# westlake-repl/IDvs.MoRec

Hardware: AMD Instinct MI355X
Metric: user-sequences/sec end-to-end train step, SASRec+BERT-base (higher is better)
Workload: dtype fp16

## Files before the change

idvs/morec_amd/_lib.py:

```python
from __future__ import annotations

import ctypes as C
import os

import torch

_HERE = os.path.dirname(os.path.abspath(__file__))
LIB_PATH = os.environ.get("MOREC_HIP_LIB") or os.path.join(_HERE, "libmorec_hip.so")

F32, BF16, F16 = 0, 1, 2
ACT_NONE, ACT_GELU, ACT_RELU = 0, 1, 2
DACT_MUL = 3


class MorecError(RuntimeError):
    pass


class GemmDesc(C.Structure):
    _fields_ = [("M", C.c_int), ("N", C.c_int), ("K", C.c_int), ("lda", C.c_int), ("ldb", C.c_int), ("ldc", C.c_int),
                ("in_dtype", C.c_int), ("out_dtype", C.c_int), ("act", C.c_int), ("dact", C.c_int),
                ("accumulate", C.c_int), ("split_k", C.c_int), ("alpha", C.c_float), ("aux_deriv", C.c_int)]


class GemmPlanInfo(C.Structure):
    _fields_ = [("family", C.c_int), ("mode", C.c_int), ("tile_rows", C.c_int), ("tile_cols", C.c_int), ("ngroup", C.c_int),
                ("colsum_fused", C.c_int), ("family_name", C.c_char_p)]


class AttnDesc(C.Structure):
    _fields_ = [("n_seq", C.c_int), ("T", C.c_int), ("n_heads", C.c_int), ("dh", C.c_int), ("causal", C.c_int),
                ("scale", C.c_float), ("mask_value", C.c_float), ("dtype", C.c_int), ("p_drop", C.c_float),
                ("seed", C.c_uint64), ("cu_seqlens", C.c_void_p), ("total_rows", C.c_int), ("spare_rows_max", C.c_int)]


class TransposeItem(C.Structure):
    _fields_ = [("src", C.c_void_p), ("dst", C.c_void_p), ("rows", C.c_int), ("cols", C.c_int), ("ld_src", C.c_int),
                ("ld_dst", C.c_int), ("tile0", C.c_int), ("reserved", C.c_int)]


class CeDesc(C.Structure):
    _fields_ = [("B", C.c_int), ("S", C.c_int), ("D", C.c_int), ("Nc", C.c_int), ("col_offset", C.c_int),
                ("dtype", C.c_int), ("dE_fp32", C.c_int), ("ws_from_fwd", C.c_int)]


class StepParams(C.Structure):
    _fields_ = [("step", C.c_int32), ("found_inf", C.c_int32), ("growth_tracker", C.c_int32), ("skipped", C.c_int32),
                ("loss_scale", C.c_float), ("inv_scale", C.c_float), ("bc1", C.c_float), ("bc2", C.c_float), ("apply", C.c_int32),
                ("pad0", C.c_int32), ("drop_seed", C.c_uint64), ("drop_seed_mixed", C.c_uint64), ("reserved", C.c_int32 * 2)]


class SwinAttnDesc(C.Structure):
    _fields_ = [("n_img", C.c_int), ("H", C.c_int), ("W", C.c_int), ("window", C.c_int), ("shift", C.c_int),
                ("heads", C.c_int), ("dh", C.c_int), ("scale", C.c_float), ("dtype", C.c_int)]


_P = C.c_void_p
_SIGS = {
    "morec_strerror": (C.c_char_p, [C.c_int]),
    "morec_version": (C.c_int, []),
    "morec_tuning_set": (C.c_int, [C.c_char_p, C.c_int]),
    "morec_det_scratch_reserve": (C.c_int, [C.c_size_t, C.c_void_p]),
    "morec_stream_wait_stream": (C.c_int, [_P, _P]),
    "morec_fold_defer_begin": (C.c_int, [_P]),
    "morec_fold_defer_active": (C.c_int, []),
    "morec_fold_flush": (C.c_int, [_P]),
    "morec_fold_defer_end": (C.c_int, []),
    "morec_fold_stats": (C.c_int, [_P]),
    "morec_gemm_nt": (C.c_int, [C.POINTER(GemmDesc), _P, _P, _P, _P, _P, _P, _P]),
    "morec_gemm_nt_colsum": (C.c_int, [C.POINTER(GemmDesc), _P, _P, _P, _P, _P, _P, _P, _P, _P]),
    "morec_gemm_colsum_workspace_bytes": (C.c_size_t, [C.c_int, C.c_int]),
    "morec_gemm_plan": (C.c_int, [C.POINTER(GemmDesc), C.c_int, C.c_int, C.c_int, C.c_int, C.c_int, C.POINTER(GemmPlanInfo)]),
    "morec_gemm_tn": (C.c_int, [_P, _P, _P, C.c_int, C.c_int, C.c_int, C.c_int, C.c_int, C.c_int, C.c_int, C.c_int, C.c_int, _P, _P]),
    "morec_gemm_tn_workspace_bytes": (C.c_size_t, [C.c_int, C.c_int, C.c_int]),
    "morec_mlp_dact_recompute_supported": (C.c_int, [C.c_int, C.c_int, C.c_int, C.c_int]),
    "morec_mlp_dact_recompute_workspace_bytes": (C.c_size_t, [C.c_int]),
    "morec_mlp_dact_recompute": (C.c_int, [_P, _P, _P, _P, _P, _P, _P, _P, C.c_int, C.c_int, C.c_int, C.c_int, _P]),
    "morec_transpose": (C.c_int, [_P, _P, C.c_int, C.c_int, C.c_int, C.c_int, C.c_int, C.c_int, _P]),
    "morec_transpose_batch": (C.c_int, [_P, C.c_int, C.c_int, C.c_int, _P]),
    "morec_cast": (C.c_int, [_P, _P, C.c_size_t, C.c_int, C.c_int, _P]),
    "morec_split_bf16x3": (C.c_int, [_P, _P, C.c_int, C.c_int, C.c_int, C.c_int, C.c_int, _P]),
    "morec_act_bwd": (C.c_int, [_P, _P, _P, C.c_size_t, C.c_int, C.c_int, _P]),
    "morec_scaled_sum": (C.c_int, [_P, _P, _P, _P, C.c_size_t, C.c_float, C.c_int, _P]),
    "morec_colsum": (C.c_int, [_P, _P, C.c_int, C.c_int, C.c_int, C.c_int, _P]),
    "morec_layernorm_fwd": (C.c_int, [_P, _P, _P, _P, C.c_int, _P, _P, C.c_float, _P, _P, _P, _P, C.c_int, C.c_int,
                                      C.c_int, C.c_float, C.c_uint64, C.c_float, C.c_uint64, _P, C.c_int, _P]),
    "morec_layernorm_bwd": (C.c_int, [_P, _P, _P, _P, _P, _P, _P, _P, _P, _P, _P, C.c_int, C.c_int, C.c_int, C.c_float,
                                      C.c_uint64, C.c_float, C.c_uint64, _P, _P, C.c_int, _P]),
    "morec_layernorm_fwd_res32": (C.c_int, [_P, _P, _P, _P, C.c_int, _P, _P, C.c_float, _P, _P, _P, _P, _P, C.c_int, C.c_int,
                                            C.c_int, C.c_float, C.c_uint64, C.c_float, C.c_uint64, _P]),
    "morec_layernorm_fwd_res32_pre": (C.c_int, [_P, _P, _P, _P, _P, _P, _P, _P, _P, C.c_float, _P, _P, _P, _P, C.c_int, C.c_int, C.c_int,
                                                C.c_float, C.c_uint64, _P]),
    "morec_layernorm_bwd_res32": (C.c_int, [_P, _P, _P, _P, _P, _P, _P, _P, _P, _P, _P, C.c_int, C.c_int, C.c_int, C.c_float,
                                            C.c_uint64, C.c_float, C.c_uint64, _P]),
    "morec_pos_grad": (C.c_int, [_P, _P, C.c_int, C.c_int, C.c_int, C.c_int, _P]),
    "morec_attn_fwd": (C.c_int, [C.POINTER(AttnDesc), _P, _P, _P, _P]),
    "morec_attn_bwd": (C.c_int, [C.POINTER(AttnDesc), _P, _P, _P, _P, _P]),
    "morec_attn_bwd_dbias": (C.c_int, [C.POINTER(AttnDesc), _P, _P, _P, _P, C.c_int, _P, _P, C.c_size_t, _P]),
    "morec_bert_embed_fwd": (C.c_int, [_P, _P, _P, _P, _P, _P, C.c_float, _P, _P, _P, _P, C.c_int, C.c_int, C.c_int,
                                       C.c_int, C.c_float, C.c_uint64, _P]),
    "morec_bert_embed_bwd": (C.c_int, [_P, _P, _P, _P, _P, C.c_int, C.c_int, C.c_int, C.c_int, C.c_int, _P, _P]),
    "morec_gather_rows": (C.c_int, [_P, _P, _P, C.c_int, C.c_int, C.c_int, _P]),
    "morec_scatter_add_rows": (C.c_int, [_P, _P, _P, C.c_int, C.c_int, C.c_int, C.c_int, _P]),
    "morec_indexed_rows_copy": (C.c_int, [_P, _P, _P, _P, C.c_int, C.c_int, C.c_int, _P]),
    "morec_strided_rows_copy": (C.c_int, [_P, _P, C.c_int, C.c_int, C.c_int, C.c_int, C.c_int, _P]),
    "morec_inbatch_ce_workspace_bytes": (C.c_size_t, [C.POINTER(CeDesc)]),
    "morec_inbatch_ce_fwd": (C.c_int, [C.POINTER(CeDesc), _P, _P, _P, _P, _P, _P, _P, _P, _P, _P, _P, _P]),
    "morec_inbatch_ce_bwd": (C.c_int, [C.POINTER(CeDesc), _P, _P, _P, _P, _P, _P, _P, _P, _P, C.c_float, _P, _P, _P,
                                       _P]),
    "morec_bce_fwd": (C.c_int, [_P, _P, _P, _P, _P, C.c_int, C.c_int, C.c_int, C.c_int, _P]),
    "morec_bce_bwd": (C.c_int, [_P, _P, _P, _P, _P, _P, _P, C.c_int, C.c_int, C.c_int, C.c_int, _P]),
    "morec_adamw": (C.c_int, [_P, _P, _P, _P, _P, C.c_size_t, C.c_float, C.c_float, C.c_float, C.c_float, C.c_float,
                              C.c_int, C.c_float, _P]),
    "morec_dropout_seed_source": (C.c_int, [_P]),
    "morec_step_params_init": (C.c_int, [_P, C.c_float, C.c_int, _P]),
    "morec_grad_check_finite": (C.c_int, [_P, C.c_size_t, _P, _P]),
    "morec_step_decide": (C.c_int, [_P, C.c_float, C.c_float, C.c_float, C.c_float, C.c_int, C.c_int, _P]),
    "morec_adamw_sp": (C.c_int, [_P, _P, _P, _P, _P, C.c_int, C.c_size_t, C.c_float, C.c_float, C.c_float, C.c_float, C.c_float, _P, _P]),
    "morec_eval_rank": (C.c_int, [_P, _P, _P, C.c_int, _P, _P, _P, C.c_int, C.c_int, C.c_int, _P]),
    "morec_eval_rank_cand": (C.c_int, [_P, _P, _P, C.c_int, _P, C.c_int, _P, _P, _P, C.c_int, C.c_int, C.c_int, _P]),
    "morec_eval_topk": (C.c_int, [_P, _P, _P, C.c_int, C.c_int, C.c_int, _P, _P, _P, C.c_size_t, C.c_int, C.c_int, C.c_int, _P]),
    "morec_eval_topk_ws_bytes": (C.c_size_t, [C.c_int, C.c_int, C.c_int, C.c_int]),
    "morec_eval_topk_max_k": (C.c_int, []),
    "morec_dropout_keep_mask": (C.c_int, [_P, C.c_size_t, C.c_float, C.c_uint64, _P]),
    "morec_probe": (C.c_int, [_P, _P]),
    "morec_swin_attn_fwd": (C.c_int, [C.POINTER(SwinAttnDesc), _P, _P, _P, _P]),
    "morec_swin_attn_bwd": (C.c_int, [C.POINTER(SwinAttnDesc), _P, _P, _P, _P, _P, _P, _P]),
    "morec_swin_attn_bwd_dbias": (C.c_int, [C.POINTER(SwinAttnDesc), _P, _P, _P, _P, _P, _P, _P, _P, C.c_size_t, _P]),
    "morec_swin_bias_expand": (C.c_int, [_P, _P, C.c_int, C.c_int, _P]),
    "morec_swin_bias_reduce": (C.c_int, [_P, _P, C.c_int, C.c_int, _P]),
    "morec_swin_patchify": (C.c_int, [_P, _P, C.c_int, C.c_int, C.c_int, C.c_int, C.c_int, C.c_int, _P]),
    "morec_swin_patchify_u8": (C.c_int, [_P, _P, C.c_int, C.c_int, C.c_int, C.c_int, C.c_int, C.c_float, C.c_float, C.c_int, _P]),
    "morec_swin_merge": (C.c_int, [_P, _P, C.c_int, C.c_int, C.c_int, C.c_int, C.c_int, C.c_int, _P]),
    "morec_swin_pool_fwd": (C.c_int, [_P, _P, C.c_int, C.c_int, C.c_int, C.c_int, _P]),
    "morec_swin_pool_bwd": (C.c_int, [_P, _P, C.c_int, C.c_int, C.c_int, C.c_int, _P]),
    "morec_bias_residual": (C.c_int, [_P, _P, _P, _P, C.c_int, _P, C.c_int, C.c_int, C.c_int, _P]),
    "morec_droppath_scale": (C.c_int, [_P, C.c_int, C.c_float, C.c_uint64, _P]),
    "morec_image_resize_u8": (C.c_int, [_P, _P, _P, _P, C.c_int, C.c_int, _P]),
    "morec_comm_available": (C.c_int, []),
    "morec_comm_unique_id": (C.c_int, [_P]),
    "morec_comm_create": (C.c_int, [C.POINTER(_P), _P, C.c_int, C.c_int]),
    "morec_comm_destroy": (C.c_int, [_P]),
    "morec_comm_last_error": (C.c_char_p, [_P]),
    "morec_comm_all_gather": (C.c_int, [_P, _P, _P, C.c_size_t, _P]),
    "morec_comm_reduce_scatter_f32": (C.c_int, [_P, _P, _P, C.c_size_t, _P]),
    "morec_comm_all_reduce_f32": (C.c_int, [_P, _P, C.c_size_t, _P]),
}

EXPORTS = tuple(_SIGS)
_lib = None


def lib():
    global _lib
    if _lib is None:
        if not os.path.exists(LIB_PATH):
            raise MorecError(f"{LIB_PATH} not found: build it with `python -c 'import __graft_entry__ as g; g.build()'` "
                             "or `make -C idvs/morec_amd/csrc` -- there is no CPU/PyTorch fallback path")
        h = C.CDLL(LIB_PATH)
        for name, (res, args) in _SIGS.items():
            fn = getattr(h, name)
            fn.restype, fn.argtypes = res, args
        _lib = h
        h.morec_tuning_set(b"deterministic", int(env_flag("MOREC_DETERMINISTIC")))
    return _lib


def env_flag(name: str) -> bool:
    return os.environ.get(name, "0").strip().lower() not in ("", "0", "false", "no", "off")


def check(rc: int, what: str):
    if rc != 0:
        msg = lib().morec_strerror(rc)
        raise MorecError(f"{what} failed: rc={rc} ({msg.decode() if msg else '?'})")
```

idvs/morec_amd/csrc/gemm_tn8p.hip:

```cpp
#include "gemm_core.hpp"
#include "gemm_args.hpp"


namespace {
typedef __attribute__((ext_vector_type(16))) float f32x16_t;
typedef __attribute__((ext_vector_type(4))) unsigned int u32x4_t;
typedef __attribute__((ext_vector_type(4))) short s16x4_t;
typedef __attribute__((ext_vector_type(8))) short s16x8_t;
typedef __attribute__((address_space(3))) s16x4_t* lds_s16x4_ptr;

constexpr int TT = 64;
constexpr int ROWB = 256;
constexpr int HALF_BYTES = TT * ROWB;
constexpr int OP_BYTES = 2 * HALF_BYTES;
constexpr int BUF_BYTES = 2 * OP_BYTES;
constexpr int LDS_MAIN = 2 * BUF_BYTES;
constexpr int SLICE = 4096;
constexpr int LDS_TOTAL = LDS_MAIN + 8 * SLICE;
constexpr int THREADS = 512;

struct TnArgs8 {
    const bf16* DY;
    const bf16* X;
    float* out;
    int M, N, K, ldy, ldx, ldo, mchunk, tiles_n, tiles_k, zs;
    size_t slab_stride;
};

template <int N>
__device__ __forceinline__ void vm_wait() {
    asm volatile("s_waitcnt vmcnt(%0)" ::"n"(N) : "memory");
}
__device__ __forceinline__ void pin() { __builtin_amdgcn_sched_barrier(0); }
__device__ __forceinline__ void bar() {
    pin();
    __builtin_amdgcn_s_barrier();
    pin();
}
template <int REM, int W1, int W0>
__device__ __forceinline__ void vm_wait_tail() {
    vm_wait<(REM >= 2 ? 8 : (REM == 1 ? W1 : W0))>();
}

struct Ctx {
    __amdgpu_buffer_rsrc_t ry, rx;
    uint32_t y1[2], y2[2], x1[2], x2[2];
    int tok[2];
    int dpiece;
    int ay[2], ax;
    uint32_t vmask;
};

__device__ __forceinline__ void dma2(__amdgpu_buffer_rsrc_t rs, const uint32_t (&o)[2], const int (&tok)[2], int left, int soff, char* dst) {
    const uint32_t o0 = tok[0] < left ? o[0] : 0x80000000u;
    const uint32_t o1 = tok[1] < left ? o[1] : 0x80000000u;
    __builtin_amdgcn_raw_ptr_buffer_load_lds(rs, (lptr_t)dst, 16, o0, soff, 0, 0);
    __builtin_amdgcn_raw_ptr_buffer_load_lds(rs, (lptr_t)(dst + 1024), 16, o1, soff, 0, 0);
}

__device__ __forceinline__ bf16x8_t tr_frag(const char* smem, int addr, int ks) {
    const s16x4_t lo = __builtin_amdgcn_ds_read_tr16_b64_v4i16((lds_s16x4_ptr)(smem + addr + (16 * ks) * ROWB));
    const s16x4_t hi = __builtin_amdgcn_ds_read_tr16_b64_v4i16((lds_s16x4_ptr)(smem + addr + (16 * ks + 4) * ROWB));
    const s16x8_t v = {lo[0], lo[1], lo[2], lo[3], hi[0], hi[1], hi[2], hi[3]};
    return __builtin_bit_cast(bf16x8_t, v);
}

template <typename T16, int N0, int KQ, bool SKIP>
__device__ __forceinline__ void mfma_quadrant(f32x16_t (&acc)[4][2], const bf16x8_t (&fy)[2][4], const bf16x8_t (&fx)[4], uint32_t vm) {
    if constexpr (SKIP) {
        if (!(vm & (16u << KQ))) return;
        const bool a = (vm >> N0) & 1u, b = (vm >> (N0 + 1)) & 1u;
        if (!(a && b)) {
            if (!(a || b)) return;
            __builtin_amdgcn_s_setprio(1);
            if (a) {
#pragma unroll
                for (int ks = 0; ks < 4; ++ks) acc[N0][KQ] = h16<T16>::mma32(fx[ks], fy[0][ks], acc[N0][KQ]);
            } else {
#pragma unroll
                for (int ks = 0; ks < 4; ++ks) acc[N0 + 1][KQ] = h16<T16>::mma32(fx[ks], fy[1][ks], acc[N0 + 1][KQ]);
            }
            __builtin_amdgcn_s_setprio(0);
            return;
        }
    }
    __builtin_amdgcn_s_setprio(1);
#pragma unroll
    for (int ks = 0; ks < 4; ++ks)
#pragma unroll
        for (int ni = 0; ni < 2; ++ni)
            acc[N0 + ni][KQ] = h16<T16>::mma32(fx[ks], fy[ni][ks], acc[N0 + ni][KQ]);
    __builtin_amdgcn_s_setprio(0);
}

template <typename T16, int REM, bool SKIP>
__device__ __forceinline__ void stage(char* smem, const Ctx& c, int cb, int soy, int sox, int dy_step, int dx_step, int left,
                                      f32x16_t (&acc)[4][2]) {
    char* cur = smem + cb;
    char* oth = smem + (cb ^ BUF_BYTES);
    bf16x8_t fy[2][4], fx0[4], fx1[4];
    const int ay0 = cb + c.ay[0], ay1 = cb + c.ay[1], ax = cb + OP_BYTES + c.ax;
#pragma unroll
    for (int ks = 0; ks < 4; ++ks) fx0[ks] = tr_frag(smem, ax, ks);
#pragma unroll
    for (int ks = 0; ks < 4; ++ks) {
        fy[0][ks] = tr_frag(smem, ay0, ks);
        fy[1][ks] = tr_frag(smem, ay1, ks);
    }
    if constexpr (REM >= 1) dma2(c.rx, c.x2, c.tok, left - TT, sox + dx_step, oth + OP_BYTES + HALF_BYTES + c.dpiece);
    pin();
    vm_wait_tail<REM, 8, 2>();
    bar();
    mfma_quadrant<T16, 0, 0, SKIP>(acc, fy, fx0, c.vmask);
    bar();
#pragma unroll
    for (int ks = 0; ks < 4; ++ks) fx1[ks] = tr_frag(smem, ax + HALF_BYTES, ks);
    if constexpr (REM >= 1) dma2(c.ry, c.y2, c.tok, left - TT, soy + dy_step, oth + HALF_BYTES + c.dpiece);
    pin();
    vm_wait_tail<REM, 8, 0>();
    bar();
    mfma_quadrant<T16, 0, 1, SKIP>(acc, fy, fx1, c.vmask);
    bar();
#pragma unroll
    for (int ks = 0; ks < 4; ++ks) {
        fy[0][ks] = tr_frag(smem, ay0 + HALF_BYTES, ks);
        fy[1][ks] = tr_frag(smem, ay1 + HALF_BYTES, ks);
    }
    if constexpr (REM >= 2) dma2(c.ry, c.y1, c.tok, left - 2 * TT, soy + 2 * dy_step, cur + c.dpiece);
    pin();
    vm_wait_tail<REM, 6, 0>();
    bar();
    mfma_quadrant<T16, 2, 1, SKIP>(acc, fy, fx1, c.vmask);
    bar();
    if constexpr (REM >= 2) dma2(c.rx, c.x1, c.tok, left - 2 * TT, sox + 2 * dx_step, cur + OP_BYTES + c.dpiece);
    pin();
    vm_wait_tail<REM, 4, 0>();
    bar();
    mfma_quadrant<T16, 2, 0, SKIP>(acc, fy, fx0, c.vmask);
    bar();
}

template <typename T16, bool SKIP>
__device__ __forceinline__ void tn_body(const TnArgs8& p, char* smem, const bf16* __restrict__ DYt, const bf16* __restrict__ Xt, int n0, int k0,
                                        int mbeg, int mend, float* __restrict__ dst) {
    const int lane = threadIdx.x & 63;
    const int wave = __builtin_amdgcn_readfirstlane(threadIdx.x >> 6);
    const int wr = wave >> 2, wc = wave & 3;
    const int nt = (mend - mbeg + TT - 1) / TT;
    Ctx c;
    {
#pragma unroll
        for (int j = 0; j < 2; ++j) {
            const int t = 8 * wave + 4 * j + (lane >> 4);
            const int lc = (lane & 15) ^ (4 * (t & 3));
            const int ycol = (lc < 8 ? lc * 8 : 128 + (lc - 8) * 8);
            const int xcol = (lc >> 2) * 64 + (lc & 3) * 8;
            c.tok[j] = t;
            c.y1[j] = (uint32_t)(t * p.ldy + min(n0 + ycol, p.N - 8) - n0) * 2u;
            c.y2[j] = (uint32_t)(t * p.ldy + min(n0 + ycol + 64, p.N - 8) - n0) * 2u;
            c.x1[j] = (uint32_t)(t * p.ldx + min(k0 + xcol, p.K - 8) - k0) * 2u;
            c.x2[j] = (uint32_t)(t * p.ldx + min(k0 + xcol + 32, p.K - 8) - k0) * 2u;
        }
        const long ybytes = (long)(p.M - mbeg) * p.ldy * 2, xbytes = (long)(p.M - mbeg) * p.ldx * 2;
        c.ry = __builtin_amdgcn_make_buffer_rsrc((void*)DYt, 0, (int)min(ybytes, 0x7fffffffL), 0x00020000);
        c.rx = __builtin_amdgcn_make_buffer_rsrc((void*)Xt, 0, (int)min(xbytes, 0x7fffffffL), 0x00020000);
        c.dpiece = 8 * wave * ROWB;
        const int rr = (lane & 15) >> 2, cgrp = (lane >> 4) & 1, h = lane >> 5;
        const int rowoff = (8 * h + rr) * ROWB + 8 * (lane & 3);
#pragma unroll
        for (int cg = 0; cg < 2; ++cg) c.ay[cg] = rowoff + (((wr * 4 + cg * 2 + cgrp) ^ (2 * rr)) << 5);
        c.ax = rowoff + (((wc * 2 + cgrp) ^ (2 * rr)) << 5);
        uint32_t vm = 0;
#pragma unroll
        for (int i = 0; i < 4; ++i) vm |= (n0 + wr * 128 + i * 32 < p.N) ? (1u << i) : 0u;
#pragma unroll
        for (int j = 0; j < 2; ++j) vm |= (k0 + wc * 64 + j * 32 < p.K) ? (16u << j) : 0u;
        c.vmask = __builtin_amdgcn_readfirstlane(vm);
    }
    const int dy_step = TT * p.ldy * 2, dx_step = TT * p.ldx * 2;
    const int left0 = mend - mbeg;
    dma2(c.ry, c.y1, c.tok, left0, 0, smem + c.dpiece);
    dma2(c.rx, c.x1, c.tok, left0, 0, smem + OP_BYTES + c.dpiece);
    dma2(c.rx, c.x2, c.tok, left0, 0, smem + OP_BYTES + HALF_BYTES + c.dpiece);
    dma2(c.ry, c.y2, c.tok, left0, 0, smem + HALF_BYTES + c.dpiece);
    dma2(c.ry, c.y1, c.tok, left0 - TT, dy_step, smem + BUF_BYTES + c.dpiece);
    dma2(c.rx, c.x1, c.tok, left0 - TT, dx_step, smem + BUF_BYTES + OP_BYTES + c.dpiece);
    pin();

    f32x16_t acc[4][2];
#pragma unroll
    for (int i = 0; i < 4; ++i)
#pragma unroll
        for (int j = 0; j < 2; ++j)
#pragma unroll
            for (int v = 0; v < 16; ++v) acc[i][j][v] = 0.f;
    vm_wait<8>();
    bar();
    if (wr == 1) bar();
    int cb = 0, t = 0;
    for (; t < nt - 2; ++t) {
        stage<T16, 2, SKIP>(smem, c, cb, t * dy_step, t * dx_step, dy_step, dx_step, left0 - t * TT, acc);
        cb ^= BUF_BYTES;
    }
    stage<T16, 1, SKIP>(smem, c, cb, t * dy_step, t * dx_step, dy_step, dx_step, left0 - t * TT, acc);
    stage<T16, 0, SKIP>(smem, c, cb ^ BUF_BYTES, (t + 1) * dy_step, (t + 1) * dx_step, dy_step, dx_step, left0 - (t + 1) * TT, acc);
    if (wr == 0) bar();

    const int r5 = lane & 31, hh = lane >> 5;
    char* ws = smem + LDS_MAIN + wave * SLICE;
    const int rs_row = lane >> 3, rs_slot = lane & 7;
    const int rs_off = rs_row * 128 + ((rs_slot ^ (rs_row & 7)) << 4);
    const int nrows = min(256, p.N - n0);
    const long obytes = (long)nrows * p.ldo * 4;
    const __amdgpu_buffer_rsrc_t ro = __builtin_amdgcn_make_buffer_rsrc((void*)(dst + (size_t)n0 * p.ldo), 0, (int)min(obytes, 0x7fffffffL), 0x00020000);
    auto wfence = [&]() {
        __builtin_amdgcn_fence(__ATOMIC_RELEASE, "wavefront");
        __builtin_amdgcn_wave_barrier();
        __builtin_amdgcn_fence(__ATOMIC_ACQUIRE, "wavefront");
    };
#pragma unroll
    for (int Ni = 0; Ni < 4; ++Ni) {
#pragma unroll
        for (int Ki = 0; Ki < 2; ++Ki) {
            pin();
#pragma unroll
            for (int g = 0; g < 4; ++g) {
                const int slot = 2 * g + hh;
                *reinterpret_cast<float4*>(ws + r5 * 128 + ((slot ^ (r5 & 7)) << 4)) =
                    make_float4(acc[Ni][Ki][4 * g], acc[Ni][Ki][4 * g + 1], acc[Ni][Ki][4 * g + 2], acc[Ni][Ki][4 * g + 3]);
            }
            wfence();
            u32x4_t q[4];
#pragma unroll
            for (int i = 0; i < 4; ++i) q[i] = *reinterpret_cast<const u32x4_t*>(ws + rs_off + i * 1024);
            const int kcol = k0 + wc * 64 + Ki * 32 + rs_slot * 4;
            const uint32_t lo = kcol < p.K ? (uint32_t)((rs_row * p.ldo + kcol) * 4) : 0x80000000u;
#pragma unroll
            for (int i = 0; i < 4; ++i)
                __builtin_amdgcn_raw_buffer_store_b128(q[i], ro, lo + (uint32_t)((wr * 128 + Ni * 32 + 8 * i) * p.ldo * 4), 0, 0);
            wfence();
        }
    }
}

template <typename T16, bool SKIP>
__global__ __launch_bounds__(THREADS) void gemm_tn8p_kernel(TnArgs8 p) {
    extern __shared__ __attribute__((aligned(16))) char smem[];
    const int tiles = p.tiles_n * p.tiles_k;
    const int item = xcd_remap(blockIdx.x, tiles * p.zs);
    const int z = item / tiles, wg = item - z * tiles;
    const int n0 = (wg / p.tiles_k) * 256, k0 = (wg % p.tiles_k) * 256;
    const int mbeg = z * p.mchunk, mend = min(p.M, mbeg + p.mchunk);
    tn_body<T16, SKIP>(p, smem, p.DY + (size_t)mbeg * p.ldy + n0, p.X + (size_t)mbeg * p.ldx + k0, n0, k0, mbeg, mend,
            p.out + (size_t)z * p.slab_stride);
}
}

int gemm_tn8p_try_launch(const bf16* DY, const bf16* X, float* out, size_t slab_stride, int M, int N, int K, int ldy, int ldx, int ldo,
                         int mchunk, int zs, int dtype, hipStream_t s) {
    const int mode = tuning().gemm8p;
    if (mode == 1) return MOREC_E_UNSUPPORTED;
    if (N % 8 || K % 8 || ldo % 4) return MOREC_E_UNSUPPORTED;
    if (mchunk % TT || mchunk < 2 * TT) return MOREC_E_UNSUPPORTED;
    if (M - (zs - 1) * (long)mchunk < 2 * TT && zs > 1) return MOREC_E_UNSUPPORTED;
    if (zs == 1 && M < 2 * TT) return MOREC_E_UNSUPPORTED;
    const int tiles_n = (N + 255) / 256, tiles_k = (K + 255) / 256;
    if (mode != 2) {
        if (mchunk < 8 * TT) return MOREC_E_UNSUPPORTED;
    }
    if ((long)M * ldy * 2 >= 0x7fffffffL || (long)M * ldx * 2 >= 0x7fffffffL) return MOREC_E_UNSUPPORTED;
    TnArgs8 a;
    a.DY = DY; a.X = X; a.out = out; a.M = M; a.N = N; a.K = K; a.ldy = ldy; a.ldx = ldx; a.ldo = ldo; a.mchunk = mchunk;
    a.tiles_n = tiles_n; a.tiles_k = tiles_k; a.zs = zs; a.slab_stride = slab_stride;
    if (!by_h16(dtype, [&](auto* t) {
            using T = MOREC_TAG_T(t);
            static const hipError_t attr_rc = hipFuncSetAttribute(reinterpret_cast<const void*>(&gemm_tn8p_kernel<T, false>), hipFuncAttributeMaxDynamicSharedMemorySize, LDS_TOTAL);
            static const hipError_t attr_rc2 = hipFuncSetAttribute(reinterpret_cast<const void*>(&gemm_tn8p_kernel<T, true>), hipFuncAttributeMaxDynamicSharedMemorySize, LDS_TOTAL);
            (void)attr_rc; (void)attr_rc2;
            if (tuning().tn8p_skip && ((N % 256 != 0 && N % 256 <= 224) || (K % 256 != 0 && K % 256 <= 224)))
                hipLaunchKernelGGL((gemm_tn8p_kernel<T, true>), dim3(tiles_n * tiles_k * zs), dim3(THREADS), LDS_TOTAL, s, a);
            else
                hipLaunchKernelGGL((gemm_tn8p_kernel<T, false>), dim3(tiles_n * tiles_k * zs), dim3(THREADS), LDS_TOTAL, s, a);
        }))
        return MOREC_E_UNSUPPORTED;
    MOREC_CHECK_LAUNCH();
    return MOREC_OK;
}
```

idvs/morec_amd/csrc/tuning.hip:

```cpp
#include <stdlib.h>
#include <string.h>
#include "common.hpp"

namespace {
enum Handling {
    RAW,
    FLAG,
    TMR,
    RESERVE,
    TAIL_BIAS,
    MFMA,
    AT_LEAST_1,
    NOT_CHAR_0,
    IS_CHAR_1,
    EPI,
};
struct Row {
    const char* key;
    const char* env;
    int Tuning::*field;
    int def;
    Handling how;
};
const Row ROWS[] = {
    {"gemm8p", "MOREC_GEMM8P", &Tuning::gemm8p, 0, RAW},
    {"gemm2w", "MOREC_GEMM2W", &Tuning::gemm2w, 0, RAW},
    {"gemm_small", "MOREC_GEMM_SMALL", &Tuning::gemm_small, 0, RAW},
    {"gemm_skinny", "MOREC_GEMM_SKINNY", &Tuning::gemm_skinny, 0, RAW},
    {"ce8p", "MOREC_CE8P", &Tuning::ce8p, 0, RAW},
    {"gemm8p_tmr", "MOREC_GEMM8P_TMR", &Tuning::gemm8p_tmr, 1, TMR},
    {"gemm8p_ngroup", "MOREC_GEMM8P_NGROUP", &Tuning::gemm8p_ngroup, -1, RAW},
    {"gemm8p_reserve_cus", "MOREC_GEMM8P_RESERVE_CUS", &Tuning::gemm8p_reserve_cus, 0, RESERVE},
    {"gemm8p_tail_split", "MOREC_GEMM8P_TAIL_SPLIT", &Tuning::gemm8p_tail_split, 0, FLAG},
    {"gemm8p_tail_bias", nullptr, &Tuning::gemm8p_tail_bias, 2, TAIL_BIAS},
    {"gemm8p_mfma", "MOREC_GEMM8P_MFMA", &Tuning::gemm8p_mfma, 0, MFMA},
    {"gemm8p_debug", "MOREC_GEMM8P_DEBUG", &Tuning::gemm8p_debug, 0, RAW},
    {"gemm8p_stamps_lo", nullptr, &Tuning::gemm8p_stamps_lo, 0, RAW},
    {"gemm8p_stamps_hi", nullptr, &Tuning::gemm8p_stamps_hi, 0, RAW},
    {"deterministic", "MOREC_DETERMINISTIC", &Tuning::deterministic, 0, FLAG},
    {"fold_defer", "MOREC_FOLD_DEFER", &Tuning::fold_defer, 1, FLAG},
    {nullptr, "MOREC_GEMM_TILE", &Tuning::gemm_tile, 0, RAW},
    {nullptr, "MOREC_GEMM_EPI", &Tuning::gemm_epi, 2, EPI},
    {nullptr, "MOREC_GEMM2W_STAGGER", &Tuning::gemm2w_stagger, 0, RAW},
    {nullptr, "MOREC_TN8P_SKIP", &Tuning::tn8p_skip, 1, FLAG},
    {nullptr, "MOREC_ATTN_MFMA64", &Tuning::attn_mfma64, 1, NOT_CHAR_0},
    {nullptr, "MOREC_ATTN_F32_MFMA", &Tuning::attn_f32_mfma, 1, NOT_CHAR_0},
    {nullptr, "MOREC_SWIN_WPW_MIN", &Tuning::swin_wpw_min, 8, AT_LEAST_1},
    {nullptr, "MOREC_SWIN_BWD_WIDE", &Tuning::swin_bwd_wide, 1, RAW},
    {nullptr, "MOREC_QUIET", &Tuning::quiet, 0, IS_CHAR_1},
};

int handled(Handling how, int v) {
    switch (how) {
        case FLAG: return v != 0;
        case TMR: return (v == 0 || v == 1 || v == 224 || v == 192) ? v : 1;
        case RESERVE: return v < 0 ? 0 : v > 128 ? 128 : v;
        case TAIL_BIAS: return v < 0 ? 0 : v > 16 ? 16 : v;
        case MFMA: return (v == 16 || v == 32) ? v : 0;
        case AT_LEAST_1: return v < 1 ? 1 : v;
        default: return v;
    }
}

Tuning& table() {
    static Tuning t = [] {
        Tuning x{};
        for (const Row& r : ROWS) {
            const char* e = r.env ? getenv(r.env) : nullptr;
            x.*r.field = !e                    ? r.def
                         : r.how == NOT_CHAR_0 ? e[0] != '0'
                         : r.how == IS_CHAR_1  ? e[0] == '1'
                         : r.how == EPI        ? e[0] == 'w'
                                               : handled(r.how, atoi(e));
        }
        return x;
    }();
    return t;
}
}

const Tuning& tuning() { return table(); }

extern "C" int morec_tuning_set(const char* key, int value) {
    if (!key) return MOREC_E_ARG;
    for (const Row& r : ROWS)
        if (r.key && !strcmp(key, r.key)) {
            if (r.how == MFMA && value != 0 && value != 16 && value != 32) return MOREC_E_UNSUPPORTED;
            table().*r.field = handled(r.how, value);
            return MOREC_OK;
        }
    return MOREC_E_UNSUPPORTED;
}

bool morec_deterministic() { return tuning().deterministic != 0; }
void morec_set_deterministic(int on) { table().deterministic = on ? 1 : 0; }

int device_cu_count() {
    static const int n = [] {
        int dev = 0, c = 0;
        (void)hipGetDevice(&dev);
        if (hipDeviceGetAttribute(&c, hipDeviceAttributeMultiprocessorCount, dev) != hipSuccess || c <= 0) c = 256;
        return c;
    }();
    return n;
}

int gemm8p_cu_count() {
    const int n_dev = device_cu_count() & ~7;
    const int n = (n_dev < 8 ? 8 : n_dev) - (tuning().gemm8p_reserve_cus & ~7);
    return n < 8 ? 8 : n;
}
```

idvs/morec_amd/csrc/tuning.hpp:

```cpp
#pragma once

struct Tuning {
    int gemm8p, gemm2w, gemm_small, gemm_skinny, ce8p;
    int gemm8p_tmr;
    int gemm8p_ngroup;
    int gemm8p_reserve_cus;
    int gemm8p_tail_split, gemm8p_tail_bias;
    int gemm8p_mfma;
    int gemm8p_debug;
    int gemm8p_stamps_lo, gemm8p_stamps_hi;
    int deterministic;
    int fold_defer;
    int gemm_tile;
    int gemm_epi;
    int gemm2w_stagger;
    int tn8p_skip;
    int attn_mfma64;
    int attn_f32_mfma;
    int swin_wpw_min;
    int swin_bwd_wide;
    int quiet;

    unsigned long long gemm8p_stamps() const {
        return ((unsigned long long)(unsigned)gemm8p_stamps_hi << 32) | (unsigned)gemm8p_stamps_lo;
    }
};

const Tuning& tuning();

int device_cu_count();
int gemm8p_cu_count();
```

include/morec_hip.h:

```cpp
#ifndef MOREC_HIP_H
#define MOREC_HIP_H

#include <stddef.h>
#include <stdint.h>

#ifdef __cplusplus
extern "C" {
#endif

#define MOREC_F32 0
#define MOREC_BF16 1
#define MOREC_F16 2

#define MOREC_OK 0
#define MOREC_E_ARG (-1)
#define MOREC_E_ALIGN (-2)
#define MOREC_E_UNSUPPORTED (-3)
#define MOREC_E_DTYPE (-4)
#define MOREC_E_COMM (-5)

#define MOREC_ACT_NONE 0
#define MOREC_ACT_GELU 1
#define MOREC_ACT_RELU 2
#define MOREC_DACT_MUL 3

const char* morec_strerror(int code);
int morec_version(void);
int morec_tuning_set(const char* key, int value);
int morec_det_scratch_reserve(size_t n_floats, void* stream);
int morec_fold_defer_begin(void* stream);
int morec_fold_defer_active(void);
int morec_fold_flush(void* run_on);
int morec_fold_defer_end(void);
int morec_fold_stats(unsigned long long* out4);

typedef struct {
    int M, N, K;
    int lda, ldb, ldc;
    int in_dtype;
    int out_dtype;
    int act;
    int dact;
    int accumulate;
    int split_k;
    float alpha;
    int aux_deriv;
} morec_gemm_desc;

int morec_gemm_nt(const morec_gemm_desc* d, const void* A, const void* B, void* C, const float* bias,
                  void* aux_out, const void* dact_in, void* stream);

size_t morec_gemm_colsum_workspace_bytes(int M, int N);
int morec_gemm_nt_colsum(const morec_gemm_desc* d, const void* A, const void* B, void* C, const float* bias,
                         void* aux_out, const void* dact_in, float* colsum_out, float* workspace, void* stream);

#define MOREC_GEMM_UNSUPPORTED 0
#define MOREC_GEMM_SKINNY 1
#define MOREC_GEMM_SKINNY_WIDE 2
#define MOREC_GEMM_TWO_W 3
#define MOREC_GEMM_EIGHT_P 4
#define MOREC_GEMM_SMALL 5
#define MOREC_GEMM_GENERIC 6
typedef struct {
    int family;
    int mode;
    int tile_rows, tile_cols;
    int ngroup;
    int colsum_fused;
    const char* family_name;
} morec_gemm_plan_info;
int morec_gemm_plan(const morec_gemm_desc* d, int has_bias, int has_aux, int has_dact_in, int has_colsum, int n_cu,
                    morec_gemm_plan_info* out);

int morec_mlp_dact_recompute_supported(int M, int N, int K, int dtype);
size_t morec_mlp_dact_recompute_workspace_bytes(int N);
int morec_mlp_dact_recompute(const void* dY, const void* W2t, const void* X, const void* W1, const float* b1, void* dU,
                             float* colsum_out, float* workspace, int M, int N, int K, int dtype, void* stream);

int morec_gemm_tn(const void* DY, const void* X, float* C, int M, int N, int K, int ldy, int ldx, int ldc, int dtype,
                  int split_m, int accumulate, float* workspace, void* stream);
size_t morec_gemm_tn_workspace_bytes(int N, int K, int split_m);

int morec_transpose(const void* in, void* out, int R, int C, int ld_in, int ld_out, int in_dtype, int out_dtype,
                    void* stream);

typedef struct {
    const void* src;
    void* dst;
    int rows, cols;
    int ld_src, ld_dst;
    int tile0;
    int reserved;
} morec_transpose_item;
int morec_transpose_batch(const morec_transpose_item* items, int n_items, int n_tiles, int dtype, void* stream);
int morec_cast(const void* in, void* out, size_t n, int in_dtype, int out_dtype, void* stream);
int morec_split_bf16x3(const float* in, void* out, int R, int C, int ld_in, int ld_out, int lo_slot, void* stream);
int morec_act_bwd(const void* dy, const void* pre, void* out, size_t n, int act, int dtype, void* stream);
int morec_scaled_sum(const void* x0, const void* x1, const void* x2, void* out, size_t n, float scale, int dtype, void* stream);
int morec_colsum(const void* in, float* out, int M, int N, int ld, int dtype, void* stream);

int morec_layernorm_fwd(const void* x, const float* bias, const void* res, const float* pos, int pos_period,
                        const float* gamma, const float* beta, float eps, void* z_out, void* y, float* mean,
                        float* rstd, int M, int N, int dtype, float p_in, uint64_t seed_in, float p_out,
                        uint64_t seed_out, const float* rowscale, int rows_per_scale, void* stream);
int morec_layernorm_bwd(const void* dy_a, const void* dy_b, const void* z, const float* mean, const float* rstd,
                        const float* gamma, void* dz, void* dzd, float* dgamma, float* dbeta, float* dbias, int M, int N,
                        int dtype, float p_in, uint64_t seed_in, float p_out, uint64_t seed_out, const void* dres,
                        const float* rowscale, int rows_per_scale, void* stream);

int morec_layernorm_fwd_res32(const void* x16, const float* bias, const float* res32, const float* pos, int pos_period, const float* gamma,
                              const float* beta, float eps, float* z32, float* y32, void* y16, float* mean, float* rstd, int M, int N,
                              int dtype16, float p_in, uint64_t seed_in, float p_out, uint64_t seed_out, void* stream);
int morec_layernorm_fwd_res32_pre(const void* x16, const float* bias, const float* res_z32, const float* res_mean, const float* res_rstd,
                                  const float* res_gamma, const float* res_beta, const float* gamma, const float* beta, float eps, float* z32,
                                  void* y16, float* mean, float* rstd, int M, int N, int dtype16, float p_in, uint64_t seed_in, void* stream);
int morec_layernorm_bwd_res32(const void* dy16, const float* dy32, const float* z32, const float* mean, const float* rstd, const float* gamma,
                              float* dz32, void* dzd16, float* dgamma, float* dbeta, float* dbias, int M, int N, int dtype16, float p_in,
                              uint64_t seed_in, float p_out, uint64_t seed_out, void* stream);
int morec_pos_grad(const void* dz, float* dpos, int M, int N, int period, int dtype, void* stream);

typedef struct {
    int n_seq, T, n_heads, dh;
    int causal;
    float scale, mask_value;
    int dtype;
    float p_drop;
    uint64_t seed;
    const int32_t* cu_seqlens;
    int total_rows;
    int spare_rows_max;
} morec_attn_desc;

int morec_attn_fwd(const morec_attn_desc* d, const void* qkv, const float* key_keep, void* ctx, void* stream);
int morec_attn_bwd(const morec_attn_desc* d, const void* qkv, const float* key_keep, const void* dctx, void* dqkv,
                   void* stream);
int morec_attn_bwd_dbias(const morec_attn_desc* d, const void* qkv, const float* key_keep, const void* dctx, void* dqkv,
                         int rows, float* dbias, float* ws, size_t ws_bytes, void* stream);

typedef struct {
    int n_img, H, W;
    int window;
    int shift;
    int heads, dh;
    float scale;
    int dtype;
} morec_swin_attn_desc;
int morec_swin_attn_fwd(const morec_swin_attn_desc* d, const void* qkv, const float* bias_t, void* ctx, void* stream);
int morec_swin_attn_bwd(const morec_swin_attn_desc* d, const void* qkv, const float* bias_t, const void* ctx,
                        const void* dctx, void* dqkv, float* dbias_t, void* stream);
int morec_swin_attn_bwd_dbias(const morec_swin_attn_desc* d, const void* qkv, const float* bias_t, const void* ctx,
                              const void* dctx, void* dqkv, float* dbias_t, float* dbqkv, float* ws, size_t ws_bytes, void* stream);
int morec_swin_bias_expand(const float* table, float* bias_t, int window, int heads, void* stream);
int morec_swin_bias_reduce(const float* dbias_t, float* dtable, int window, int heads, void* stream);
int morec_swin_patchify(const float* pixels, void* out, int n_img, int channels, int R, int patch, int ld_out, int dtype,
                        void* stream);
int morec_swin_patchify_u8(const uint8_t* pixels_hwc, void* out, int n_img, int channels, int R, int patch, int ld_out,
                           float mean, float std, int dtype, void* stream);
int morec_swin_merge(const void* in, void* out, int n_img, int H, int W, int C, int reverse, int dtype, void* stream);
int morec_swin_pool_fwd(const void* x, void* out, int n_img, int tokens, int C, int dtype, void* stream);
int morec_swin_pool_bwd(const void* dout, void* dx, int n_img, int tokens, int C, int dtype, void* stream);
int morec_bias_residual(const void* a, const float* bias, const void* res, const float* rowscale, int rows_per_scale,
                        void* out, int M, int N, int dtype, void* stream);
int morec_droppath_scale(float* out, int n, float p, uint64_t seed, void* stream);

int morec_bce_fwd(const void* P, const void* E, const uint8_t* row_valid, float* scores, float* loss_sum, int B, int S, int D,
                  int dtype, void* stream);
int morec_bce_bwd(const void* P, const void* E, const uint8_t* row_valid, const float* scores, const float* gscale, void* dP,
                  void* dE, int B, int S, int D, int dtype, void* stream);

int morec_bert_embed_fwd(const int32_t* ids, const float* word, const float* pos, const float* type0,
                         const float* gamma, const float* beta, float eps, void* z_out, void* y, float* mean,
                         float* rstd, int M, int T, int H, int dtype, float p_out, uint64_t seed_out, void* stream);
int morec_bert_embed_bwd(const int32_t* ids, const void* dz, float* dword, float* dpos, float* dtype0, int pad_id,
                         int M, int T, int H, int dtype, const int32_t* order, void* stream);
int morec_gather_rows(const float* table, const int32_t* idx, void* out, int R, int D, int dtype, void* stream);
int morec_scatter_add_rows(const void* d, const int32_t* idx, float* dtable, int R, int D, int pad_id, int dtype,
                           void* stream);
int morec_indexed_rows_copy(const void* in, void* out, const int32_t* in_idx, const int32_t* out_idx, int R, int D, int dtype,
                            void* stream);
int morec_strided_rows_copy(const void* in, void* out, int R, int D, int in_row_stride, int out_row_stride,
                            int dtype, void* stream);
// ... 80 lines not shown
```

Baseline: 3676.

## Add 16x16 MFMA variant to TN weight-gradient GEMM with heuristic selection

Templates the tn8p weight-gradient GEMM kernel on MFMA shape, adding a 16x16x16 path next to the existing 32x32x8 path. The new path brings its own LDS fragment addressing with an extra swizzle, split accumulator blocks and a remapped epilogue. A heuristic picks 16x16 when chunk tokens are at least 1024 and K is at least 192, and an env/tuning knob can force either shape. The intent is better MFMA throughput or LDS read efficiency on large-M backward GEMMs, at the cost of more instructions and different bank-conflict behaviour.

```diff
diff --git a/idvs/morec_amd/_lib.py b/idvs/morec_amd/_lib.py
--- a/idvs/morec_amd/_lib.py
+++ b/idvs/morec_amd/_lib.py
@@ -60,6 +60,7 @@
     "morec_strerror": (C.c_char_p, [C.c_int]),
     "morec_version": (C.c_int, []),
     "morec_tuning_set": (C.c_int, [C.c_char_p, C.c_int]),
+    "morec_gemm_tn8p_mfma": (C.c_int, [C.c_int, C.c_int]),
     "morec_det_scratch_reserve": (C.c_int, [C.c_size_t, C.c_void_p]),
     "morec_stream_wait_stream": (C.c_int, [_P, _P]),
     "morec_fold_defer_begin": (C.c_int, [_P]),
diff --git a/idvs/morec_amd/csrc/gemm_tn8p.hip b/idvs/morec_amd/csrc/gemm_tn8p.hip
--- a/idvs/morec_amd/csrc/gemm_tn8p.hip
+++ b/idvs/morec_amd/csrc/gemm_tn8p.hip
@@ -42,12 +42,14 @@
     vm_wait<(REM >= 2 ? 8 : (REM == 1 ? W1 : W0))>();
 }
 
+template <int MF>
 struct Ctx {
+    static constexpr int NB = MF == 16 ? 2 : 1;
     __amdgpu_buffer_rsrc_t ry, rx;
     uint32_t y1[2], y2[2], x1[2], x2[2];
     int tok[2];
     int dpiece;
-    int ay[2], ax;
+    int ay[2][NB], ax[NB];
     uint32_t vmask;
 };
 
@@ -58,15 +60,80 @@
     __builtin_amdgcn_raw_ptr_buffer_load_lds(rs, (lptr_t)(dst + 1024), 16, o1, soff, 0, 0);
 }
 
+template <int KT>
 __device__ __forceinline__ bf16x8_t tr_frag(const char* smem, int addr, int ks) {
-    const s16x4_t lo = __builtin_amdgcn_ds_read_tr16_b64_v4i16((lds_s16x4_ptr)(smem + addr + (16 * ks) * ROWB));
-    const s16x4_t hi = __builtin_amdgcn_ds_read_tr16_b64_v4i16((lds_s16x4_ptr)(smem + addr + (16 * ks + 4) * ROWB));
+    const s16x4_t lo = __builtin_amdgcn_ds_read_tr16_b64_v4i16((lds_s16x4_ptr)(smem + addr + (KT * ks) * ROWB));
+    const s16x4_t hi = __builtin_amdgcn_ds_read_tr16_b64_v4i16((lds_s16x4_ptr)(smem + addr + (KT * ks + 4) * ROWB));
     const s16x8_t v = {lo[0], lo[1], lo[2], lo[3], hi[0], hi[1], hi[2], hi[3]};
     return __builtin_bit_cast(bf16x8_t, v);
 }
-
-template <typename T16, int N0, int KQ, bool SKIP>
-__device__ __forceinline__ void mfma_quadrant(f32x16_t (&acc)[4][2], const bf16x8_t (&fy)[2][4], const bf16x8_t (&fx)[4], uint32_t vm) {
+template <int MF>
+__device__ __forceinline__ void frags_x(bf16x8_t (&f)[4], const char* smem, const int (&a)[MF == 16 ? 2 : 1], int half) {
+    if constexpr (MF == 32) {
+#pragma unroll
+        for (int ks = 0; ks < 4; ++ks) f[ks] = tr_frag<16>(smem, a[0] + half, ks);
+    } else {
+#pragma unroll
+        for (int b = 0; b < 2; ++b)
+#pragma unroll
+            for (int ks = 0; ks < 2; ++ks) f[2 * b + ks] = tr_frag<32>(smem, a[b] + half, ks);
+    }
+}
+template <int MF>
+__device__ __forceinline__ void frags_y(bf16x8_t (&f)[2][4], const char* smem, const int (&a)[2][MF == 16 ? 2 : 1], int half) {
+    if constexpr (MF == 32) {
+#pragma unroll
+        for (int ks = 0; ks < 4; ++ks) {
+            f[0][ks] = tr_frag<16>(smem, a[0][0] + half, ks);
+            f[1][ks] = tr_frag<16>(smem, a[1][0] + half, ks);
+        }
+    } else {
+#pragma unroll
+        for (int b = 0; b < 2; ++b)
+#pragma unroll
+            for (int ks = 0; ks < 2; ++ks) {
+                f[0][2 * b + ks] = tr_frag<32>(smem, a[0][b] + half, ks);
+                f[1][2 * b + ks] = tr_frag<32>(smem, a[1][b] + half, ks);
+            }
+    }
+}
+
+struct Blk16 { f32x4_t s[4]; };
+template <int MF> struct BlkOf { typedef f32x16_t type; };
+template <> struct BlkOf<16> { typedef Blk16 type; };
+template <int MF> using blk_t = typename BlkOf<MF>::type;
+
+template <typename T16, int MF>
+__device__ __forceinline__ blk_t<MF> mma_step(blk_t<MF> blk, const bf16x8_t (&fx)[4], const bf16x8_t (&fy)[4], int ks) {
+    if constexpr (MF == 32) {
+        return h16<T16>::mma32(fx[ks], fy[ks], blk);
+    } else {
+#pragma unroll
+        for (int sb = 0; sb < 4; ++sb) blk.s[sb] = h16<T16>::mma16(fx[2 * (sb & 1) + ks], fy[2 * (sb >> 1) + ks], blk.s[sb]);
+        return blk;
+    }
+}
+template <int MF>
+__device__ __forceinline__ float4 blk_get4(const blk_t<MF>& b, int g) {
+    if constexpr (MF == 32) return make_float4(b[4 * g], b[4 * g + 1], b[4 * g + 2], b[4 * g + 3]);
+    else return make_float4(b.s[g][0], b.s[g][1], b.s[g][2], b.s[g][3]);
+}
+template <int MF>
+__device__ __forceinline__ void blk_zero(blk_t<MF>& b) {
+    if constexpr (MF == 32) {
+#pragma unroll
+        for (int v = 0; v < 16; ++v) b[v] = 0.f;
+    } else {
+#pragma unroll
+        for (int g = 0; g < 4; ++g)
+#pragma unroll
+            for (int v = 0; v < 4; ++v) b.s[g][v] = 0.f;
+    }
+}
+
+template <typename T16, int N0, int KQ, bool SKIP, int MF>
+__device__ __forceinline__ void mfma_quadrant(blk_t<MF> (&acc)[4][2], const bf16x8_t (&fy)[2][4], const bf16x8_t (&fx)[4], uint32_t vm) {
+    static_assert(MF == 32 || MF == 16, "MFMA shape");
     if constexpr (SKIP) {
         if (!(vm & (16u << KQ))) return;
         const bool a = (vm >> N0) & 1u, b = (vm >> (N0 + 1)) & 1u;
@@ -75,10 +142,10 @@
             __builtin_amdgcn_s_setprio(1);
             if (a) {
 #pragma unroll
-                for (int ks = 0; ks < 4; ++ks) acc[N0][KQ] = h16<T16>::mma32(fx[ks], fy[0][ks], acc[N0][KQ]);
+                for (int ks = 0; ks < (MF == 32 ? 4 : 2); ++ks) acc[N0][KQ] = mma_step<T16, MF>(acc[N0][KQ], fx, fy[0], ks);
             } else {
 #pragma unroll
-                for (int ks = 0; ks < 4; ++ks) acc[N0 + 1][KQ] = h16<T16>::mma32(fx[ks], fy[1][ks], acc[N0 + 1][KQ]);
+                for (int ks = 0; ks < (MF == 32 ? 4 : 2); ++ks) acc[N0 + 1][KQ] = mma_step<T16, MF>(acc[N0 + 1][KQ], fx, fy[1], ks);
             }
             __builtin_amdgcn_s_setprio(0);
             return;
@@ -86,73 +153,69 @@
     }
     __builtin_amdgcn_s_setprio(1);
 #pragma unroll
-    for (int ks = 0; ks < 4; ++ks)
-#pragma unroll
-        for (int ni = 0; ni < 2; ++ni)
-            acc[N0 + ni][KQ] = h16<T16>::mma32(fx[ks], fy[ni][ks], acc[N0 + ni][KQ]);
+    for (int ks = 0; ks < (MF == 32 ? 4 : 2); ++ks)
+#pragma unroll
+        for (int ni = 0; ni < 2; ++ni) acc[N0 + ni][KQ] = mma_step<T16, MF>(acc[N0 + ni][KQ], fx, fy[ni], ks);
     __builtin_amdgcn_s_setprio(0);
 }
 
-template <typename T16, int REM, bool SKIP>
-__device__ __forceinline__ void stage(char* smem, const Ctx& c, int cb, int soy, int sox, int dy_step, int dx_step, int left,
-                                      f32x16_t (&acc)[4][2]) {
+template <typename T16, int REM, bool SKIP, int MF>
+__device__ __forceinline__ void stage(char* smem, const Ctx<MF>& c, int cb, int soy, int sox, int dy_step, int dx_step, int left,
+                                      blk_t<MF> (&acc)[4][2]) {
     char* cur = smem + cb;
     char* oth = smem + (cb ^ BUF_BYTES);
     bf16x8_t fy[2][4], fx0[4], fx1[4];
-    const int ay0 = cb + c.ay[0], ay1 = cb + c.ay[1], ax = cb + OP_BYTES + c.ax;
-#pragma unroll
-    for (int ks = 0; ks < 4; ++ks) fx0[ks] = tr_frag(smem, ax, ks);
-#pragma unroll
-    for (int ks = 0; ks < 4; ++ks) {
-        fy[0][ks] = tr_frag(smem, ay0, ks);
-        fy[1][ks] = tr_frag(smem, ay1, ks);
-    }
+    constexpr int NB = Ctx<MF>::NB;
+    int ay[2][NB], ax[NB];
+#pragma unroll
+    for (int b = 0; b < NB; ++b) {
+        ay[0][b] = cb + c.ay[0][b];
+        ay[1][b] = cb + c.ay[1][b];
+        ax[b] = cb + OP_BYTES + c.ax[b];
+    }
+    frags_x<MF>(fx0, smem, ax, 0);
+    frags_y<MF>(fy, smem, ay, 0);
     if constexpr (REM >= 1) dma2(c.rx, c.x2, c.tok, left - TT, sox + dx_step, oth + OP_BYTES + HALF_BYTES + c.dpiece);
     pin();
     vm_wait_tail<REM, 8, 2>();
     bar();
-    mfma_quadrant<T16, 0, 0, SKIP>(acc, fy, fx0, c.vmask);
-    bar();
-#pragma unroll
-    for (int ks = 0; ks < 4; ++ks) fx1[ks] = tr_frag(smem, ax + HALF_BYTES, ks);
+    mfma_quadrant<T16, 0, 0, SKIP, MF>(acc, fy, fx0, c.vmask);
+    bar();
+    frags_x<MF>(fx1, smem, ax, HALF_BYTES);
     if constexpr (REM >= 1) dma2(c.ry, c.y2, c.tok, left - TT, soy + dy_step, oth + HALF_BYTES + c.dpiece);
     pin();
     vm_wait_tail<REM, 8, 0>();
     bar();
-    mfma_quadrant<T16, 0, 1, SKIP>(acc, fy, fx1, c.vmask);
-    bar();
-#pragma unroll
-    for (int ks = 0; ks < 4; ++ks) {
-        fy[0][ks] = tr_frag(smem, ay0 + HALF_BYTES, ks);
-        fy[1][ks] = tr_frag(smem, ay1 + HALF_BYTES, ks);
-    }
+    mfma_quadrant<T16, 0, 1, SKIP, MF>(acc, fy, fx1, c.vmask);
+    bar();
+    frags_y<MF>(fy, smem, ay, HALF_BYTES);
     if constexpr (REM >= 2) dma2(c.ry, c.y1, c.tok, left - 2 * TT, soy + 2 * dy_step, cur + c.dpiece);
     pin();
     vm_wait_tail<REM, 6, 0>();
     bar();
-    mfma_quadrant<T16, 2, 1, SKIP>(acc, fy, fx1, c.vmask);
+    mfma_quadrant<T16, 2, 1, SKIP, MF>(acc, fy, fx1, c.vmask);
     bar();
     if constexpr (REM >= 2) dma2(c.rx, c.x1, c.tok, left - 2 * TT, sox + 2 * dx_step, cur + OP_BYTES + c.dpiece);
     pin();
     vm_wait_tail<REM, 4, 0>();
     bar();
-    mfma_quadrant<T16, 2, 0, SKIP>(acc, fy, fx0, c.vmask);
-    bar();
-}
-
-template <typename T16, bool SKIP>
+    mfma_quadrant<T16, 2, 0, SKIP, MF>(acc, fy, fx0, c.vmask);
+    bar();
+}
+
+template <typename T16, bool SKIP, int MF>
 __device__ __forceinline__ void tn_body(const TnArgs8& p, char* smem, const bf16* __restrict__ DYt, const bf16* __restrict__ Xt, int n0, int k0,
                                         int mbeg, int mend, float* __restrict__ dst) {
     const int lane = threadIdx.x & 63;
     const int wave = __builtin_amdgcn_readfirstlane(threadIdx.x >> 6);
     const int wr = wave >> 2, wc = wave & 3;
     const int nt = (mend - mbeg + TT - 1) / TT;
-    Ctx c;
+    Ctx<MF> c;
     {
 #pragma unroll
         for (int j = 0; j < 2; ++j) {
             const int t = 8 * wave + 4 * j + (lane >> 4);
-            const int lc = (lane & 15) ^ (4 * (t & 3));
+            const int lc = (lane & 15) ^ (4 * (t & 3)) ^ (MF == 16 ? 2 * (wave & 1) : 0);
             const int ycol = (lc < 8 ? lc * 8 : 128 + (lc - 8) * 8);
             const int xcol = (lc >> 2) * 64 + (lc & 3) * 8;
             c.tok[j] = t;
@@ -165,11 +228,23 @@
         c.ry = __builtin_amdgcn_make_buffer_rsrc((void*)DYt, 0, (int)min(ybytes, 0x7fffffffL), 0x00020000);
         c.rx = __builtin_amdgcn_make_buffer_rsrc((void*)Xt, 0, (int)min(xbytes, 0x7fffffffL), 0x00020000);
         c.dpiece = 8 * wave * ROWB;
-        const int rr = (lane & 15) >> 2, cgrp = (lane >> 4) & 1, h = lane >> 5;
+        const int rr = (lane & 15) >> 2, cgrp = (lane >> 4) & 1, h = MF == 32 ? lane >> 5 : lane >> 4;
         const int rowoff = (8 * h + rr) * ROWB + 8 * (lane & 3);
 #pragma unroll
-        for (int cg = 0; cg < 2; ++cg) c.ay[cg] = rowoff + (((wr * 4 + cg * 2 + cgrp) ^ (2 * rr)) << 5);
-        c.ax = rowoff + (((wc * 2 + cgrp) ^ (2 * rr)) << 5);
+        for (int cg = 0; cg < 2; ++cg) {
+            if constexpr (MF == 32) {
+                c.ay[cg][0] = rowoff + (((wr * 4 + cg * 2 + cgrp) ^ (2 * rr)) << 5);
+            } else {
+#pragma unroll
+                for (int b = 0; b < 2; ++b) c.ay[cg][b] = rowoff + (((wr * 4 + cg * 2 + b) ^ (2 * rr) ^ cgrp) << 5);
+            }
+        }
+        if constexpr (MF == 32) {
+            c.ax[0] = rowoff + (((wc * 2 + cgrp) ^ (2 * rr)) << 5);
+        } else {
+#pragma unroll
+            for (int b = 0; b < 2; ++b) c.ax[b] = rowoff + (((wc * 2 + b) ^ (2 * rr) ^ cgrp) << 5);
+        }
         uint32_t vm = 0;
 #pragma unroll
         for (int i = 0; i < 4; ++i) vm |= (n0 + wr * 128 + i * 32 < p.N) ? (1u << i) : 0u;
@@ -187,26 +262,24 @@
     dma2(c.rx, c.x1, c.tok, left0 - TT, dx_step, smem + BUF_BYTES + OP_BYTES + c.dpiece);
     pin();
 
-    f32x16_t acc[4][2];
+    blk_t<MF> acc[4][2];
 #pragma unroll
     for (int i = 0; i < 4; ++i)
 #pragma unroll
-        for (int j = 0; j < 2; ++j)
-#pragma unroll
-            for (int v = 0; v < 16; ++v) acc[i][j][v] = 0.f;
+        for (int j = 0; j < 2; ++j) blk_zero<MF>(acc[i][j]);
     vm_wait<8>();
     bar();
     if (wr == 1) bar();
     int cb = 0, t = 0;
     for (; t < nt - 2; ++t) {
-        stage<T16, 2, SKIP>(smem, c, cb, t * dy_step, t * dx_step, dy_step, dx_step, left0 - t * TT, acc);
+        stage<T16, 2, SKIP, MF>(smem, c, cb, t * dy_step, t * dx_step, dy_step, dx_step, left0 - t * TT, acc);
         cb ^= BUF_BYTES;
     }
-    stage<T16, 1, SKIP>(smem, c, cb, t * dy_step, t * dx_step, dy_step, dx_step, left0 - t * TT, acc);
-    stage<T16, 0, SKIP>(smem, c, cb ^ BUF_BYTES, (t + 1) * dy_step, (t + 1) * dx_step, dy_step, dx_step, left0 - (t + 1) * TT, acc);
+    stage<T16, 1, SKIP, MF>(smem, c, cb, t * dy_step, t * dx_step, dy_step, dx_step, left0 - t * TT, acc);
+    stage<T16, 0, SKIP, MF>(smem, c, cb ^ BUF_BYTES, (t + 1) * dy_step, (t + 1) * dx_step, dy_step, dx_step, left0 - (t + 1) * TT, acc);
     if (wr == 0) bar();
 
-    const int r5 = lane & 31, hh = lane >> 5;
+    const int r5 = MF == 32 ? lane & 31 : lane & 15, hh = MF == 32 ? lane >> 5 : lane >> 4;
     char* ws = smem + LDS_MAIN + wave * SLICE;
     const int rs_row = lane >> 3, rs_slot = lane & 7;
     const int rs_off = rs_row * 128 + ((rs_slot ^ (rs_row & 7)) << 4);
@@ -225,9 +298,9 @@
             pin();
 #pragma unroll
             for (int g = 0; g < 4; ++g) {
-                const int slot = 2 * g + hh;
-                *reinterpret_cast<float4*>(ws + r5 * 128 + ((slot ^ (r5 & 7)) << 4)) =
-                    make_float4(acc[Ni][Ki][4 * g], acc[Ni][Ki][4 * g + 1], acc[Ni][Ki][4 * g + 2], acc[Ni][Ki][4 * g + 3]);
+                const int slot = MF == 32 ? 2 * g + hh : 4 * (g & 1) + hh;
+                const int row = MF == 32 ? r5 : 16 * (g >> 1) + r5;
+                *reinterpret_cast<float4*>(ws + row * 128 + ((slot ^ (r5 & 7)) << 4)) = blk_get4<MF>(acc[Ni][Ki], g);
             }
             wfence();
             u32x4_t q[4];
@@ -243,7 +316,7 @@
     }
 }
 
-template <typename T16, bool SKIP>
+template <typename T16, bool SKIP, int MF>
 __global__ __launch_bounds__(THREADS) void gemm_tn8p_kernel(TnArgs8 p) {
     extern __shared__ __attribute__((aligned(16))) char smem[];
     const int tiles = p.tiles_n * p.tiles_k;
@@ -251,9 +324,23 @@
     const int z = item / tiles, wg = item - z * tiles;
     const int n0 = (wg / p.tiles_k) * 256, k0 = (wg % p.tiles_k) * 256;
     const int mbeg = z * p.mchunk, mend = min(p.M, mbeg + p.mchunk);
-    tn_body<T16, SKIP>(p, smem, p.DY + (size_t)mbeg * p.ldy + n0, p.X + (size_t)mbeg * p.ldx + k0, n0, k0, mbeg, mend,
+    tn_body<T16, SKIP, MF>(p, smem, p.DY + (size_t)mbeg * p.ldy + n0, p.X + (size_t)mbeg * p.ldx + k0, n0, k0, mbeg, mend,
             p.out + (size_t)z * p.slab_stride);
 }
+
+template <typename T16, bool SKIP, int MF>
+void launch_tn8p(const TnArgs8& a, dim3 grid, hipStream_t s) {
+    static const hipError_t attr_rc = hipFuncSetAttribute(reinterpret_cast<const void*>(&gemm_tn8p_kernel<T16, SKIP, MF>),
+                                                          hipFuncAttributeMaxDynamicSharedMemorySize, LDS_TOTAL);
+    (void)attr_rc;
+    hipLaunchKernelGGL((gemm_tn8p_kernel<T16, SKIP, MF>), grid, dim3(THREADS), LDS_TOTAL, s, a);
+}
+}
+
+extern "C" int morec_gemm_tn8p_mfma(int chunk_tokens, int K) {
+    const int forced = tuning().tn8p_mfma;
+    if (forced) return forced;
+    return (chunk_tokens >= 16 * TT && K >= 192) ? 16 : 32;
 }
 
 int gemm_tn8p_try_launch(const bf16* DY, const bf16* X, float* out, size_t slab_stride, int M, int N, int K, int ldy, int ldx, int ldo,
@@ -272,15 +359,13 @@
     TnArgs8 a;
     a.DY = DY; a.X = X; a.out = out; a.M = M; a.N = N; a.K = K; a.ldy = ldy; a.ldx = ldx; a.ldo = ldo; a.mchunk = mchunk;
     a.tiles_n = tiles_n; a.tiles_k = tiles_k; a.zs = zs; a.slab_stride = slab_stride;
+    const int mf = morec_gemm_tn8p_mfma(mchunk, K);
+    const bool skip = tuning().tn8p_skip && ((N % 256 != 0 && N % 256 <= 224) || (K % 256 != 0 && K % 256 <= 224));
+    const dim3 grid(tiles_n * tiles_k * zs);
     if (!by_h16(dtype, [&](auto* t) {
             using T = MOREC_TAG_T(t);
-            static const hipError_t attr_rc = hipFuncSetAttribute(reinterpret_cast<const void*>(&gemm_tn8p_kernel<T, false>), hipFuncAttributeMaxDynamicSharedMemorySize, LDS_TOTAL);
-            static const hipError_t attr_rc2 = hipFuncSetAttribute(reinterpret_cast<const void*>(&gemm_tn8p_kernel<T, true>), hipFuncAttributeMaxDynamicSharedMemorySize, LDS_TOTAL);
-            (void)attr_rc; (void)attr_rc2;
-            if (tuning().tn8p_skip && ((N % 256 != 0 && N % 256 <= 224) || (K % 256 != 0 && K % 256 <= 224)))
-                hipLaunchKernelGGL((gemm_tn8p_kernel<T, true>), dim3(tiles_n * tiles_k * zs), dim3(THREADS), LDS_TOTAL, s, a);
-            else
-                hipLaunchKernelGGL((gemm_tn8p_kernel<T, false>), dim3(tiles_n * tiles_k * zs), dim3(THREADS), LDS_TOTAL, s, a);
+            if (mf == 16) skip ? launch_tn8p<T, true, 16>(a, grid, s) : launch_tn8p<T, false, 16>(a, grid, s);
+            else skip ? launch_tn8p<T, true, 32>(a, grid, s) : launch_tn8p<T, false, 32>(a, grid, s);
         }))
         return MOREC_E_UNSUPPORTED;
     MOREC_CHECK_LAUNCH();
diff --git a/idvs/morec_amd/csrc/tuning.hip b/idvs/morec_amd/csrc/tuning.hip
--- a/idvs/morec_amd/csrc/tuning.hip
+++ b/idvs/morec_amd/csrc/tuning.hip
@@ -34,6 +34,7 @@
     {"gemm8p_tail_split", "MOREC_GEMM8P_TAIL_SPLIT", &Tuning::gemm8p_tail_split, 0, FLAG},
     {"gemm8p_tail_bias", nullptr, &Tuning::gemm8p_tail_bias, 2, TAIL_BIAS},
     {"gemm8p_mfma", "MOREC_GEMM8P_MFMA", &Tuning::gemm8p_mfma, 0, MFMA},
+    {"tn8p_mfma", "MOREC_TN8P_MFMA", &Tuning::tn8p_mfma, 0, MFMA},
     {"gemm8p_debug", "MOREC_GEMM8P_DEBUG", &Tuning::gemm8p_debug, 0, RAW},
     {"gemm8p_stamps_lo", nullptr, &Tuning::gemm8p_stamps_lo, 0, RAW},
     {"gemm8p_stamps_hi", nullptr, &Tuning::gemm8p_stamps_hi, 0, RAW},
diff --git a/idvs/morec_amd/csrc/tuning.hpp b/idvs/morec_amd/csrc/tuning.hpp
--- a/idvs/morec_amd/csrc/tuning.hpp
+++ b/idvs/morec_amd/csrc/tuning.hpp
@@ -7,6 +7,7 @@
     int gemm8p_reserve_cus;
     int gemm8p_tail_split, gemm8p_tail_bias;
     int gemm8p_mfma;
+    int tn8p_mfma;
     int gemm8p_debug;
     int gemm8p_stamps_lo, gemm8p_stamps_hi;
     int deterministic;
diff --git a/include/morec_hip.h b/include/morec_hip.h
--- a/include/morec_hip.h
+++ b/include/morec_hip.h
@@ -27,6 +27,7 @@
 const char* morec_strerror(int code);
 int morec_version(void);
 int morec_tuning_set(const char* key, int value);
+int morec_gemm_tn8p_mfma(int chunk_tokens, int K);
 int morec_det_scratch_reserve(size_t n_floats, void* stream);
 int morec_fold_defer_begin(void* stream);
 int morec_fold_defer_active(void);
```

Result: no change. 3705, median of 6 (+0.8%).
